# IK2277/ultimate-tictactoe-alphazero

Hardware: AMD Instinct MI355X
Metric: MCTS simulations/sec (whole node), 4096 games × 50 sims/move; 1/2/4/8 GPU (higher is better)
Workload: dtype f32 activations and accumulation; tower point GEMMs as 3-term split-f16 products on the f16 MFMA (f32-level accuracy: within 1e-5 of the reference's fp32 network); 1 GPU; 4096 concurrent self-play games per GPU x 50 sims/move, MCTS_BATCH_SIZE 8, tau 1.0, continuous self-play (finished games refilled; population aged 300 moves before warmup); one step = one move of every game; games_per_gpu=4096, sims_per_move=50, mcts_batch_size=8, aged_moves=300, eval_cache_log2=23, eval_cache_clear_every=0, lanes_per_gpu=2

## Files before the change

include/uttt_nn.h:

```cpp
#ifndef UTTT_NN_H
#define UTTT_NN_H

#include <stdint.h>

#include "uttt_engine.h"

#ifdef __cplusplus
extern "C" {
#endif

#define UTTT_HEAD_PCONV_W 0
#define UTTT_HEAD_PCONV_B (UTTT_HEAD_PCONV_W + 2 * 128)
#define UTTT_HEAD_VCONV_W (UTTT_HEAD_PCONV_B + 2)
#define UTTT_HEAD_VCONV_B (UTTT_HEAD_VCONV_W + 128)
#define UTTT_HEAD_PFC_W (UTTT_HEAD_VCONV_B + 1)
#define UTTT_HEAD_PFC_B (UTTT_HEAD_PFC_W + 81 * 162)
#define UTTT_HEAD_VFC1_W (UTTT_HEAD_PFC_B + 81)
#define UTTT_HEAD_VFC1_B (UTTT_HEAD_VFC1_W + 256 * 81)
#define UTTT_HEAD_VFC2_W (UTTT_HEAD_VFC1_B + 256)
#define UTTT_HEAD_VFC2_B (UTTT_HEAD_VFC2_W + 256)
#define UTTT_HEAD_SIZE (UTTT_HEAD_VFC2_B + 1)

int uttt_nn_stem(uttt_engine_t *eng, const float *w, const float *b, float *out);
int uttt_nn_stem_states(const uttt_state_t *states, int32_t n, const float *w, const float *b, float *out,
                        void *stream);
int uttt_nn_heads(const float *act, const float *head_weights, int32_t n, float *policy, float *value,
                  int32_t softmax, void *stream);
int uttt_nn_heads_dev(const float *act, const float *head_weights, const int32_t *n_dev, int32_t max_n,
                      float *policy, float *value, int32_t softmax, void *stream);

int uttt_nn_wino3h_weights(const float *w, uint16_t *u, float *u_scale);
int uttt_nn_conv3x3_wino3h(const float *x, const uint16_t *u, float u_scale, const float *bias,
                           const float *residual, float *y, const uint32_t *x_amax, int32_t x_amax_per_board,
                           uint32_t *y_amax, uint32_t *amax_clear, int32_t clear_count, int32_t n_boards,
                           void *stream);
int uttt_nn_conv3x3_wino3h_dev(const float *x, const uint16_t *u, float u_scale, const float *bias,
                               const float *residual, float *y, const uint32_t *x_amax, int32_t x_amax_per_board,
                               uint32_t *y_amax, uint32_t *amax_clear, int32_t clear_count, const int32_t *n_dev,
                               int32_t max_boards, void *stream);
int uttt_nn_conv3x3_wino3h_f16(const float *x, const uint16_t *u, float u_scale, const float *bias,
                               const float *residual, float *y, const uint32_t *x_amax, int32_t x_amax_per_board,
                               uint32_t *y_amax, uint32_t *amax_clear, int32_t clear_count, int32_t n_boards,
                               void *stream);
int uttt_nn_conv3x3_wino3h_f16_dev(const float *x, const uint16_t *u, float u_scale, const float *bias,
                                   const float *residual, float *y, const uint32_t *x_amax, int32_t x_amax_per_board,
                                   uint32_t *y_amax, uint32_t *amax_clear, int32_t clear_count, const int32_t *n_dev,
                                   int32_t max_boards, void *stream);
int uttt_nn_tower_wino3h_dev(float *act, int64_t act_stride, const uint16_t *u_all, const float *u_scale_all,
                             const float *bias_all, int32_t n_layers, const uint32_t *stem_amax, uint32_t *rows,
                             int32_t row_stride, uint32_t *ctl, int32_t parity, const int32_t *n_dev,
                             int32_t max_boards, void *stream);
int32_t uttt_nn_tower_ctl_words(int32_t max_boards);
int uttt_nn_wino3h_set_split(int32_t split);
int uttt_nn_amax(const float *x, int64_t count, uint32_t *amax, void *stream);

#ifdef __cplusplus
}
#endif

#endif
```

ultimate-tictactoe-alphazero_amd/csrc/wino3h_conv.hip:

```cpp
#include <hip/hip_runtime.h>

#include <cmath>
#include <cstdint>

#include "uttt_nn.h"
#include "wino3h_impl.h"

namespace uttt {
void set_error(const char *fmt, ...);
}

namespace uttt {
namespace wino3h {
__global__ __launch_bounds__(256) void k_amax(const float *__restrict__ x, int64_t count, uint32_t *__restrict__ amax) {
    float m = 0.0f;
    for (int64_t i = (int64_t)blockIdx.x * 256 + threadIdx.x; i < count; i += (int64_t)gridDim.x * 256)
        m = fmaxf(m, fabsf(x[i]));
#pragma unroll
    for (int off = 32; off > 0; off >>= 1) m = fmaxf(m, __shfl_xor(m, off));
    if ((threadIdx.x & 63) == 0) atomicMax(amax, __builtin_bit_cast(uint32_t, m));
}

}
}
// ... 5 lines not shown
int uttt_nn_wino3h_weights(const float *w, uint16_t *u, float *u_scale) {
    if (!w || !u || !u_scale) {
        set_error("uttt_nn_wino3h_weights: null pointer");
        return UTTT_ERR_ARG;
    }
    static const double G[5][3] = {{0.5, 0, 0},
                                   {-0.5, -0.5, -0.5},
                                   {-1.0 / 6, 1.0 / 6, -1.0 / 6},
                                   {1.0 / 6, 1.0 / 3, 2.0 / 3},
                                   {0, 0, 1}};
    using namespace wino3h;
    double *U = new double[(size_t)NP * C * C];
    double umax = 0.0;
    for (int co = 0; co < C; ++co)
        for (int ci = 0; ci < C; ++ci) {
            const float *g = w + ((size_t)co * C + ci) * 9;
            double tg[5][3];
            for (int p = 0; p < 5; ++p)
                for (int k = 0; k < 3; ++k)
                    tg[p][k] = G[p][0] * g[0 * 3 + k] + G[p][1] * g[1 * 3 + k] + G[p][2] * g[2 * 3 + k];
            for (int p = 0; p < 5; ++p)
                for (int q = 0; q < 5; ++q) {
                    const double v = tg[p][0] * G[q][0] + tg[p][1] * G[q][1] + tg[p][2] * G[q][2];
                    U[((size_t)(p * 5 + q) * C + ci) * C + co] = v;
                    umax = fabs(v) > umax ? fabs(v) : umax;
                }
        }
    if (!std::isfinite(umax)) {
        delete[] U;
        set_error("uttt_nn_wino3h_weights: non-finite weights");
        return UTTT_ERR_ARG;
    }
    int e = 0;
    if (umax > 0.0) {
        frexp(umax, &e);
        e = 15 - e;
    }
    const double su = ldexp(1.0, e);
    for (int xi = 0; xi < NP; ++xi)
        for (int ci = 0; ci < C; ++ci)
            for (int co = 0; co < C; ++co) {
                const double v = U[((size_t)xi * C + ci) * C + co] * su;
                const _Float16 hi = (_Float16)v;
                const _Float16 lo = (_Float16)(v - (double)hi);
                const size_t o = ((size_t)xi * NCH + ci / KC) * 2 * C * 32 +
                                 ((((co / 16) * 4 + (ci % KC) / 8) * 16 + co % 16) * 8 + ci % 8);
                u[o] = __builtin_bit_cast(uint16_t, hi);
                u[o + C * 4 * 8] = __builtin_bit_cast(uint16_t, lo);
            }
    delete[] U;
    *u_scale = (float)su;
    return UTTT_OK;
}

static int conv3x3_wino3h(const float *x, const uint16_t *u, float u_scale, const float *bias, const float *residual,
                          float *y, const uint32_t *x_amax, int32_t x_amax_per_board, uint32_t *y_amax,
                          uint32_t *amax_clear, int32_t clear_count, int32_t n_boards, const int32_t *n_dev,
                          void *stream, bool f16 = false) {
    if (!x || !u || !bias || !y || !x_amax || n_boards < 0 || x == y || (residual && residual == y) ||
        !(u_scale > 0.0f) || clear_count < 0 || (clear_count > 0 && !amax_clear) ||
        (amax_clear && (amax_clear == y_amax || amax_clear == x_amax))) {
        set_error("uttt_nn_conv3x3_wino3h: bad arguments (x_amax required; output must not alias input or residual; "
                  "the cleared max row must differ from x_amax and y_amax)");
        return UTTT_ERR_ARG;
    }
    if (n_boards == 0 && clear_count == 0) return UTTT_OK;
    const int pb = x_amax_per_board ? 1 : 0;
    const int split = wino3h::split_for(n_boards > 0 ? n_boards : 1);
    if (split > 1) {
        const dim3 sgrid((unsigned)(wino3h::n_sets(n_boards > 0 ? n_boards : 1) * split));
        const hipStream_t s = (hipStream_t)stream;
#define UTTT_WINO3S(RES, SP, R, M)                                                                                 \
    hipLaunchKernelGGL((wino3h::k_wino3s_conv<RES, SP, 3, M>), sgrid, dim3(64 * (8 / SP)), 0, s, x, u, u_scale, bias, R, \
                       y, x_amax, pb, y_amax, amax_clear, clear_count, n_boards, n_dev)
        if (f16) {
            if (residual) UTTT_WINO3S(true, 2, residual, wino3h::kF16);
            else UTTT_WINO3S(false, 2, nullptr, wino3h::kF16);
        } else {
            if (residual) UTTT_WINO3S(true, 2, residual, 0);
            else UTTT_WINO3S(false, 2, nullptr, 0);
        }
#undef UTTT_WINO3S
        hipError_t r = hipGetLastError();
        if (r != hipSuccess) {
            set_error("k_wino3s_conv launch: %s", hipGetErrorString(r));
            return UTTT_ERR_HIP;
        }
        return UTTT_OK;
    }
    const dim3 grid(wino3h::grid_size(n_boards > 0 ? n_boards : 1));
    const hipStream_t st = (hipStream_t)stream;
    using wino3h::k_wino3h_conv;
    if (f16) {
        if (residual)
            hipLaunchKernelGGL((k_wino3h_conv<true, wino3h::kF16>), grid, dim3(wino3h::NT), 0, st, x, u, u_scale, bias,
                               residual, y, x_amax, pb, y_amax, amax_clear, clear_count, n_boards, n_dev);
        else
            hipLaunchKernelGGL((k_wino3h_conv<false, wino3h::kF16>), grid, dim3(wino3h::NT), 0, st, x, u, u_scale, bias,
                               nullptr, y, x_amax, pb, y_amax, amax_clear, clear_count, n_boards, n_dev);
    } else if (residual) {
        hipLaunchKernelGGL(k_wino3h_conv<true>, grid, dim3(wino3h::NT), 0, st, x, u, u_scale, bias, residual, y, x_amax,
                           pb, y_amax, amax_clear, clear_count, n_boards, n_dev);
    } else {
        hipLaunchKernelGGL(k_wino3h_conv<false>, grid, dim3(wino3h::NT), 0, st, x, u, u_scale, bias, nullptr, y, x_amax,
                           pb, y_amax, amax_clear, clear_count, n_boards, n_dev);
    }
    hipError_t r = hipGetLastError();
    if (r != hipSuccess) {
        set_error("k_wino3h_conv launch: %s", hipGetErrorString(r));
        return UTTT_ERR_HIP;
    }
    return UTTT_OK;
}

int uttt_nn_conv3x3_wino3h(const float *x, const uint16_t *u, float u_scale, const float *bias, const float *residual,
                           float *y, const uint32_t *x_amax, int32_t x_amax_per_board, uint32_t *y_amax,
                           uint32_t *amax_clear, int32_t clear_count, int32_t n_boards, void *stream) {
    return conv3x3_wino3h(x, u, u_scale, bias, residual, y, x_amax, x_amax_per_board, y_amax, amax_clear, clear_count,
                          n_boards, nullptr, stream);
}

int uttt_nn_conv3x3_wino3h_dev(const float *x, const uint16_t *u, float u_scale, const float *bias,
                               const float *residual, float *y, const uint32_t *x_amax, int32_t x_amax_per_board,
                               uint32_t *y_amax, uint32_t *amax_clear, int32_t clear_count, const int32_t *n_dev,
                               int32_t max_boards, void *stream) {
    if (!n_dev) {
        set_error("uttt_nn_conv3x3_wino3h_dev: n_dev required");
        return UTTT_ERR_ARG;
    }
    return conv3x3_wino3h(x, u, u_scale, bias, residual, y, x_amax, x_amax_per_board, y_amax, amax_clear, clear_count,
                          max_boards, n_dev, stream);
}

int uttt_nn_conv3x3_wino3h_f16(const float *x, const uint16_t *u, float u_scale, const float *bias,
                               const float *residual, float *y, const uint32_t *x_amax, int32_t x_amax_per_board,
                               uint32_t *y_amax, uint32_t *amax_clear, int32_t clear_count, int32_t n_boards,
                               void *stream) {
    return conv3x3_wino3h(x, u, u_scale, bias, residual, y, x_amax, x_amax_per_board, y_amax, amax_clear, clear_count,
                          n_boards, nullptr, stream, true);
}

int uttt_nn_conv3x3_wino3h_f16_dev(const float *x, const uint16_t *u, float u_scale, const float *bias,
                                   const float *residual, float *y, const uint32_t *x_amax, int32_t x_amax_per_board,
                                   uint32_t *y_amax, uint32_t *amax_clear, int32_t clear_count, const int32_t *n_dev,
                                   int32_t max_boards, void *stream) {
    if (!n_dev) {
        set_error("uttt_nn_conv3x3_wino3h_f16_dev: n_dev required");
        return UTTT_ERR_ARG;
    }
    return conv3x3_wino3h(x, u, u_scale, bias, residual, y, x_amax, x_amax_per_board, y_amax, amax_clear, clear_count,
                          max_boards, n_dev, stream, true);
}

int uttt_nn_tower_wino3h_dev(float *act, int64_t act_stride, const uint16_t *u_all, const float *u_scale_all,
                             const float *bias_all, int32_t n_layers, const uint32_t *stem_amax, uint32_t *rows,
                             int32_t row_stride, uint32_t *ctl, int32_t parity, const int32_t *n_dev,
                             int32_t max_boards, void *stream) {
    if (!act || act_stride < (int64_t)max_boards * 81 * 128 || !u_all || !u_scale_all || !bias_all || !stem_amax ||
        !rows || !ctl || n_layers <= 0 || n_layers % 4 != 0 || max_boards < 0 || row_stride < max_boards ||
        (parity != 0 && parity != 1)) {
        set_error("uttt_nn_tower_wino3h_dev: bad arguments (three activation buffers of max_boards boards act_stride "
                  "floats apart, n_layers a positive multiple of 4, row_stride >= max_boards, parity 0 or 1)");
        return UTTT_ERR_ARG;
    }
    if (max_boards == 0) return UTTT_OK;
    static int items = -1, cus = 0;
    if (items < 0) {
        const char *e = getenv("UTTT_TOWER_ITEMS");
        items = (e && *e) ? atoi(e) : 0;
        if (items < 0) items = 0;
        int dev = 0;
        if (hipGetDevice(&dev) != hipSuccess ||
            hipDeviceGetAttribute(&cus, hipDeviceAttributeMultiprocessorCount, dev) != hipSuccess || cus <= 0)
            cus = 256;
        const char *g = getenv("UTTT_TOWER_CUS");
        if (g && *g && atoi(g) > 0 && atoi(g) < cus) cus = atoi(g);
    }
    const int max_items = n_layers * wino3h::n_sets(max_boards);
    int per = items, wgs;
    if (per == 0) {
        wgs = max_items < cus ? max_items : cus;
        per = 1 << 30;
    } else {
        wgs = (max_items + per - 1) / per;
    }
    hipLaunchKernelGGL((wino3h::k_wino3t_tower<wino3h::kHandoff>), dim3((unsigned)wgs), dim3(wino3h::NT), 0,
                       (hipStream_t)stream, act, (int64_t)act_stride, u_all, u_scale_all, bias_all, (int)n_layers,
                       stem_amax, rows, (int)row_stride, ctl, (int)uttt_nn_tower_ctl_words(row_stride), (int)parity, per,
                       (int)max_boards, n_dev);
    hipError_t r = hipGetLastError();
    if (r != hipSuccess) {
        set_error("k_wino3t_tower launch: %s", hipGetErrorString(r));
        return UTTT_ERR_HIP;
    }
    return UTTT_OK;
}

int32_t uttt_nn_tower_ctl_words(int32_t max_boards) {
    const int32_t w = wino3h::kTowerCtlDone + (max_boards + wino3h::GB - 1) / wino3h::GB;
    return (w + 31) / 32 * 32;
}

int uttt_nn_wino3h_set_split(int32_t split) {
    if (split < -1 || split > 2) {
        set_error("uttt_nn_wino3h_set_split: split must be -1 (automatic), 0/1 (the persistent kernel) or 2");
        return UTTT_ERR_ARG;
    }
    wino3h::g_split = split;
    return UTTT_OK;
}

int uttt_nn_amax(const float *x, int64_t count, uint32_t *amax, void *stream) {
    if (!x || !amax || count < 0) {
        set_error("uttt_nn_amax: bad arguments");
        return UTTT_ERR_ARG;
    }
    if (count == 0) return UTTT_OK;
    int64_t blocks = (count + 255) / 256;
    if (blocks > 1024) blocks = 1024;
    hipLaunchKernelGGL(wino3h::k_amax, dim3((unsigned)blocks), dim3(256), 0, (hipStream_t)stream, x, count, amax);
    hipError_t r = hipGetLastError();
    if (r != hipSuccess) {
        set_error("k_amax launch: %s", hipGetErrorString(r));
        return UTTT_ERR_HIP;
    }
    return UTTT_OK;
}

}
```

ultimate-tictactoe-alphazero_amd/uttt_amd/_lib.py:

```python
import ctypes
import os

import numpy as np

PKG_ROOT = os.path.dirname(os.path.dirname(os.path.abspath(__file__)))
LIB_PATH = os.environ.get("UTTT_ENGINE_LIB") or os.path.join(PKG_ROOT, "libuttt_engine.so")

UTTT_OK = 0
ERRORS = {-1: "UTTT_ERR_ARG", -2: "UTTT_ERR_HIP", -3: "UTTT_ERR_CAPACITY", -4: "UTTT_ERR_ORDER",
          -5: "UTTT_ERR_NODEVICE", -6: "UTTT_ERR_NONFINITE"}

KERNELS = {"select": 0, "apply": 1, "encode": 2, "scan": 3, "move_end": 4, "hash_eval": 5, "playout": 15, "solve": 16,
           "solve_leaves": 17,
           "select_levels": 6, "select_trees": 7, "select_max_levels_sum": 9,
           "select_trips": 10, "select_max_trips_sum": 12}


class UtttState(ctypes.Structure):

    _fields_ = [("own", ctypes.c_uint32 * 3), ("opp", ctypes.c_uint32 * 3), ("mains", ctypes.c_uint32),
                ("active", ctypes.c_int32)]


STATE_DTYPE = np.dtype([("own", "<u4", (3,)), ("opp", "<u4", (3,)), ("mains", "<u4"), ("active", "<i4")])
assert STATE_DTYPE.itemsize == ctypes.sizeof(UtttState) == 32

_P = ctypes.c_void_p
_I32 = ctypes.c_int32
_I64 = ctypes.c_int64
_F32 = ctypes.c_float
_I32P = ctypes.POINTER(ctypes.c_int32)
_I64P = ctypes.POINTER(ctypes.c_int64)
_F32P = ctypes.POINTER(ctypes.c_float)
_F64P = ctypes.POINTER(ctypes.c_double)
_U32P = ctypes.POINTER(ctypes.c_uint32)
_U64 = ctypes.c_uint64
_I8P = ctypes.POINTER(ctypes.c_int8)
_SP = ctypes.POINTER(UtttState)

SIGNATURES = {
    "uttt_last_error": (ctypes.c_char_p, []),
    "uttt_version": (ctypes.c_char_p, []),
    "uttt_state_initial": (None, [_SP]),
    "uttt_state_from_arrays": (ctypes.c_int, [_I32P, _I32P, _I32P, _I32P, _I32, _SP]),
    "uttt_state_to_arrays": (None, [_SP, _I32P, _I32P, _I32P, _I32P, _I32P]),
    "uttt_state_next": (ctypes.c_int, [_SP, _I32, _SP]),
    "uttt_state_legal_actions": (ctypes.c_int, [_SP, _I32P]),
    "uttt_state_is_lose": (ctypes.c_int, [_SP]),
    "uttt_state_is_draw": (ctypes.c_int, [_SP]),
    "uttt_state_is_done": (ctypes.c_int, [_SP]),
    "uttt_state_is_first_player": (ctypes.c_int, [_SP]),
    "uttt_state_input_hwc": (None, [_SP, _F32P]),
    "uttt_states_input_hwc": (ctypes.c_int, [_SP, _I64, _F32P]),
    "uttt_state_to_string": (ctypes.c_int, [_SP, ctypes.c_char_p, _I32]),
    "uttt_boltzman": (ctypes.c_int, [_F32P, _I32, _F32, _F32P]),
    "uttt_playout_host": (ctypes.c_int, [_SP, _I64, _I32, _U64, _I32P, _I32P]),
    "uttt_solve_host": (ctypes.c_int, [_SP, _I64, _I32, _I8P, _I8P, _I8P, _I64P, _I8P]),
    "uttt_solve_overlay_host": (ctypes.c_int, [_SP, _I64, _I32, _I32, _I32, _F32P, _I64, _F32P, _I64, _I8P]),
    "uttt_engine_create": (ctypes.c_int, [_I32, _I32, _I32, ctypes.POINTER(_P)]),
    "uttt_engine_destroy": (ctypes.c_int, [_P]),
    "uttt_engine_share_cache": (ctypes.c_int, [_P, _P]),
    "uttt_engine_own_stream": (ctypes.c_int, [_P, ctypes.POINTER(ctypes.c_void_p)]),
    "uttt_engine_set_stream": (ctypes.c_int, [_P, _P]),
    "uttt_engine_device_bytes": (ctypes.c_int64, [_P]),
    "uttt_search_begin": (ctypes.c_int, [_P, _SP, _I32, _I32, _I32]),
    "uttt_search_begin_mode": (ctypes.c_int, [_P, _SP, _I32, _I32, _I32, _I32]),
    "uttt_search_select": (ctypes.c_int, [_P, _P, _I32P]),
    "uttt_search_select_async": (ctypes.c_int, [_P]),
    "uttt_selfplay_move_begin_async": (ctypes.c_int, [_P]),
    "uttt_selfplay_move_end_async": (ctypes.c_int, [_P]),
    "uttt_selfplay_move_result": (ctypes.c_int, [_P, _I64P, _I32P]),
    "uttt_search_count_copy": (ctypes.c_int, [_P, _P]),
    "uttt_search_select_async_tag": (ctypes.c_int, [_P, ctypes.c_int32, ctypes.c_int32]),
    "uttt_search_count_ring": (ctypes.c_int, [_P, _P, _P]),
    "uttt_search_count_ptr": (ctypes.c_int, [_P, ctypes.POINTER(ctypes.c_void_p)]),
    "uttt_search_pending": (ctypes.c_int, [_P, _SP, _I32P]),
    "uttt_search_apply": (ctypes.c_int, [_P, _P, _I64, _P, _I64, _I32, _I32]),
    "uttt_eval_hash": (ctypes.c_int, [_P, _P, _I32, _P, _P]),
    "uttt_eval_hash_dev": (ctypes.c_int, [_P, _P, _P]),
    "uttt_eval_playout_dev": (ctypes.c_int, [_P, _I32, _U64, _P, _P]),
    "uttt_playouts": (ctypes.c_int, [_P, _SP, _I32, _I32, _U64, _I32P, _I32P]),
    "uttt_solve": (ctypes.c_int, [_P, _SP, _I64, _I32, _I8P, _I8P, _I8P, _I64P, _I8P]),
    "uttt_eval_solve_dev": (ctypes.c_int, [_P, _I32, _I32, _I32, _P, _I64, _P, _I64, _P]),
    "uttt_round_hash_async": (ctypes.c_int, [_P, ctypes.c_int32, ctypes.c_int32, _P, _P]),
    "uttt_rounds_hash_async": (ctypes.c_int, [_P, ctypes.c_int32, ctypes.c_int32, _P, _P, ctypes.c_int32]),
    "uttt_rounds_hash_move": (ctypes.c_int, [_P, ctypes.c_int32, ctypes.c_int32, _P, _P, ctypes.c_int32, _P, _P, _P]),
    "uttt_search_select_host": (ctypes.c_int, [_P, _P, _P, _P]),
    "uttt_search_apply_host": (ctypes.c_int, [_P, _P, ctypes.c_int64, _P, ctypes.c_int32]),
    "uttt_search_root_visits": (ctypes.c_int, [_P, _I32P, _I32P]),
    "uttt_search_scores": (ctypes.c_int, [_P, _F32, _F32P, _I32P]),
    "uttt_selfplay_begin": (ctypes.c_int, [_P, _I64, _I64, ctypes.c_uint32, _F32, _I32, _I32, _I64]),
    "uttt_selfplay_move_begin": (ctypes.c_int, [_P, _I32P]),
    "uttt_selfplay_move_end": (ctypes.c_int, [_P, _I64P]),
    "uttt_selfplay_get_rng": (ctypes.c_int, [_P, _I32, _U32P, _I32P]),
    "uttt_selfplay_set_rng": (ctypes.c_int, [_P, _I32, _U32P, _I32]),
    "uttt_selfplay_games": (ctypes.c_int, [_P, _I64P, _I64P, _I32P, _I64, _I64P]),
    "uttt_selfplay_plies": (ctypes.c_int, [_P, _SP, _F64P, ctypes.POINTER(ctypes.c_int8),
                                           ctypes.POINTER(ctypes.c_int8), _F32P, _I64, _I64P]),
    "uttt_engine_set_timing": (ctypes.c_int, [_P, _I32]),
    "uttt_engine_kernel_stats": (ctypes.c_int, [_P, _I32, ctypes.POINTER(ctypes.c_double), _I64P, _I64P]),
    "uttt_engine_reset_stats": (ctypes.c_int, [_P]),
    "uttt_engine_set_cache": (ctypes.c_int, [_P, _I32, _I32]),
    "uttt_engine_cache_clear": (ctypes.c_int, [_P]),
    "uttt_engine_cache_stats": (ctypes.c_int, [_P, _I64P, _I64P, _I64P]),
    "uttt_engine_cache_stats2": (ctypes.c_int, [_P, _I64P, _I64P, _I64P, _I64P]),
    "uttt_nn_stem": (ctypes.c_int, [_P, _P, _P, _P]),
    "uttt_nn_stem_states": (ctypes.c_int, [_P, _I32, _P, _P, _P, _P]),
    "uttt_nn_heads": (ctypes.c_int, [_P, _P, _I32, _P, _P, _I32, _P]),
    "uttt_nn_heads_dev": (ctypes.c_int, [_P, _P, _P, _I32, _P, _P, _I32, _P]),
    "uttt_nn_wino3h_weights": (ctypes.c_int, [_F32P, _P, ctypes.POINTER(ctypes.c_float)]),
    "uttt_nn_conv3x3_wino3h": (ctypes.c_int, [_P, _P, ctypes.c_float, _P, _P, _P, _P, _I32, _P, _P, _I32, _I32, _P]),
    "uttt_nn_conv3x3_wino3h_dev": (ctypes.c_int, [_P, _P, ctypes.c_float, _P, _P, _P, _P, _I32, _P, _P, _I32, _P, _I32,
                                                  _P]),
    "uttt_nn_conv3x3_wino3h_f16": (ctypes.c_int, [_P, _P, ctypes.c_float, _P, _P, _P, _P, _I32, _P, _P, _I32, _I32,
                                                  _P]),
    "uttt_nn_conv3x3_wino3h_f16_dev": (ctypes.c_int, [_P, _P, ctypes.c_float, _P, _P, _P, _P, _I32, _P, _P, _I32, _P,
                                                      _I32, _P]),
    "uttt_nn_tower_wino3h_dev": (ctypes.c_int, [_P, _I64, _P, _P, _P, _I32, _P, _P, _I32, _P, _I32, _P, _I32, _P]),
    "uttt_nn_tower_ctl_words": (ctypes.c_int32, [_I32]),
    "uttt_nn_amax": (ctypes.c_int, [_P, _I64, _P, _P]),
    "uttt_nn_wino3h_set_split": (ctypes.c_int, [_I32]),
}

_lib = None


class EngineError(RuntimeError):
    pass


def load():
    global _lib
    if _lib is None:
        import torch
        if not os.path.exists(LIB_PATH):
            raise ImportError(f"{LIB_PATH} not built: run `make -C {PKG_ROOT}` (or __graft_entry__.build())")
        lib = ctypes.CDLL(LIB_PATH)
        for name, (res, args) in SIGNATURES.items():
            fn = getattr(lib, name)
            fn.restype = res
            fn.argtypes = args
        _lib = lib
    return _lib


_diag = None


def load_diag():
    global _diag
    if _diag is None:
        load()
        path = os.path.join(os.path.dirname(LIB_PATH), "libuttt_diag.so")
        if not os.path.exists(path):
            raise ImportError(f"{path} not built: run `make -C {PKG_ROOT} diag`")
        _diag = ctypes.CDLL(path)
    return _diag


def check(rc):
    if rc != UTTT_OK:
        msg = load().uttt_last_error().decode(errors="replace")
        if rc == -1:
            raise ValueError(msg)
        raise EngineError(f"{ERRORS.get(rc, rc)}: {msg}")
    return rc


def ptr(a, ctype):
    return a.ctypes.data_as(ctypes.POINTER(ctype))
```

ultimate-tictactoe-alphazero_amd/uttt_amd/nnfast.py:

```python
import ctypes
import weakref

import torch

from . import _lib
from ._lib import check
from .engine import RoundCount
from .model import fold_bn

HEAD = {}


def _head_layout():
    if not HEAD:
        o = 0
        for name, size in (("pconv_w", 2 * 128), ("pconv_b", 2), ("vconv_w", 128), ("vconv_b", 1),
                           ("pfc_w", 81 * 162), ("pfc_b", 81), ("vfc1_w", 256 * 81), ("vfc1_b", 256),
                           ("vfc2_w", 256), ("vfc2_b", 1)):
            HEAD[name] = (o, size)
            o += size
        HEAD["size"] = o
    return HEAD


def pack_heads(net, device):
    lay = _head_layout()
    buf = torch.zeros(lay["size"], dtype=torch.float32)
    pw, pb = fold_bn(net.policy_conv, net.policy_bn)
    vw, vb = fold_bn(net.value_conv, net.value_bn)
    parts = {"pconv_w": pw.reshape(-1), "pconv_b": pb, "vconv_w": vw.reshape(-1), "vconv_b": vb,
             "pfc_w": net.policy_fc.weight.t().reshape(-1), "pfc_b": net.policy_fc.bias,
             "vfc1_w": net.value_fc1.weight.t().reshape(-1), "vfc1_b": net.value_fc1.bias,
             "vfc2_w": net.value_fc2.weight.reshape(-1), "vfc2_b": net.value_fc2.bias}
    for k, v in parts.items():
        o, n = lay[k]
        assert v.numel() == n, (k, v.numel(), n)
        buf[o:o + n] = v.detach().float().cpu()
    return buf.to(device)


def _p(t):
    return ctypes.c_void_p(t.data_ptr())


_WEIGHTS = weakref.WeakKeyDictionary()


def _fingerprint(net):
    return tuple((t.data_ptr(), t._version) for t in net.state_dict().values())


@torch.no_grad()
def _prepared_weights(net, dev, conv):
    fp = _fingerprint(net)
    per = _WEIGHTS.setdefault(net, {})
    key = (str(dev), conv)
    hit = per.get(key)
    if hit is not None and hit[0] == fp:
        return hit[1]
    sw, sb = fold_bn(net.conv_input, net.bn_input)
    out = {"stem_w": sw.permute(1, 2, 3, 0).reshape(27, 128).contiguous().to(dev),
           "stem_b": sb.contiguous().to(dev), "heads": pack_heads(net, dev), "wino": []}
    us, sus, bs = [], [], []
    for b in net.residual_blocks:
        for cv, bn in ((b.conv1, b.bn1), (b.conv2, b.bn2)):
            w, bb = fold_bn(cv, bn)
            u, su = wino3h_weights(w)
            us.append(u)
            sus.append(su)
            bs.append(bb.float())
    out["u_all"] = torch.stack(us).to(dev)
    out["bias_all"] = torch.stack(bs).contiguous().to(dev)
    out["scale_all"] = torch.tensor(sus, dtype=torch.float32, device=dev)
    for i in range(0, len(us), 2):
        out["wino"].append(((out["u_all"][i], sus[i], out["bias_all"][i]),
                            (out["u_all"][i + 1], sus[i + 1], out["bias_all"][i + 1])))
    out["stem_bound"] = float(torch.relu(out["stem_b"].double().cpu() +
                                         out["stem_w"].double().cpu().clamp_min(0).sum(0)).max())
    per[key] = (fp, out)
    return out


class FusedNetworkEvaluator:
    needs_input = False
    device_count = True
    NROW = 4

    def __init__(self, net, engine=None, max_batch=None, conv="wino3h", device=None, precision=None, tower=None):
        import os
        net = net.eval()
        if conv != "wino3h":
            raise ValueError("conv must be 'wino3h' (the split-f16 Winograd tower; the f32-MFMA kernel was retired)")
        self.conv = conv
        self.precision = precision or os.environ.get("UTTT_NN_PRECISION", "f32")
        if self.precision not in ("f32", "f16"):
            raise ValueError("precision must be 'f32' (split-f16, f32-level) or 'f16' (one f16 product)")
        self.engine = engine
        self.lib = _lib.load()
        if engine is not None:
            dev = torch.device("cuda", engine.device)
            self.max_batch = max_batch or engine.max_trees
            if self.max_batch < engine.max_trees:
                raise ValueError(f"max_batch {self.max_batch} < the engine's {engine.max_trees} trees")
        else:
            dev = torch.device(device) if device is not None else torch.device("cuda", torch.cuda.current_device())
            if max_batch is None:
                raise ValueError("max_batch is required without an engine")
            self.max_batch = max_batch
        self.device = dev
        self.nconv = 2 * len(net.residual_blocks)
        if self.nconv % self.NROW:
            raise ValueError("the max-row rotation needs a multiple of 4 convolutions")
        w = _prepared_weights(net, dev, conv)
        self.stem_w, self.stem_b, self.heads, self.wino = w["stem_w"], w["stem_b"], w["heads"], w["wino"]
        self.u_all, self.bias_all, self.scale_all = w["u_all"], w["bias_all"], w["scale_all"]
        self.tower = tower or os.environ.get("UTTT_NN_TOWER", "layers")
        if self.tower not in ("dataflow", "layers"):
            raise ValueError("tower must be 'dataflow' (one persistent launch) or 'layers' (a launch per conv)")
        if self.precision == "f16":
            self.tower = "layers"
        self.act = torch.zeros((3, self.max_batch, 81, 128), dtype=torch.float32, device=dev)
        self.buf = [self.act[0], self.act[1], self.act[2]]
        self.ctl = torch.zeros(2 * self.lib.uttt_nn_tower_ctl_words(self.max_batch), dtype=torch.int32, device=dev)
        self.ctl_parity = 0
        self.stem_bound = w["stem_bound"]
        self.stem_amax = torch.tensor([self.stem_bound], dtype=torch.float32, device=dev).view(torch.int32)
        self.bamax = torch.zeros((self.NROW, self.max_batch), dtype=torch.int32, device=dev)
        self.policy = torch.zeros((self.max_batch, 81), dtype=torch.float32, device=dev)
        self.value = torch.zeros((self.max_batch,), dtype=torch.float32, device=dev)
        self.states = None
        self.tower_events = None

    def _stream(self):
        return ctypes.c_void_p(torch.cuda.current_stream(self.device).cuda_stream)

    @torch.no_grad()
    def forward(self, n, softmax=True):
        check(self.lib.uttt_nn_stem(self.engine.h, _p(self.stem_w), _p(self.stem_b), _p(self.buf[0])))
        if isinstance(n, RoundCount):
            return self._tower_heads(n, softmax, n_dev=self.engine.count_ptr())
        return self._tower_heads(n, softmax)

    @torch.no_grad()
    def forward_states(self, states, softmax=True):
        import numpy as np
        n = len(states)
        if n > self.max_batch:
            raise ValueError(f"{n} states > max_batch {self.max_batch}")
        if self.states is None:
            self.states = torch.zeros((self.max_batch, 8), dtype=torch.int32, device=self.device)
        if n == 0:
            return self.policy[:0], self.value[:0]
        st = np.ascontiguousarray(states).view(np.int32).reshape(n, 8)
        self.states[:n].copy_(torch.from_numpy(st))
        check(self.lib.uttt_nn_stem_states(_p(self.states), n, _p(self.stem_w), _p(self.stem_b), _p(self.buf[0]),
                                           self._stream()))
        return self._tower_heads(n, softmax)

    def _dev_plan(self, stream, n_dev):
        key = (stream.value, n_dev.value)
        if getattr(self, "_plan", None) is None or self._plan[0] != key:
            rows = [ctypes.c_void_p(self.bamax[r].data_ptr()) for r in range(self.NROW)]
            cap = self.max_batch
            x, t, y = (ctypes.c_void_p(b.data_ptr()) for b in self.buf)
            calls, i = [], 0
            for (u1, s1, b1), (u2, s2, b2) in self.wino:
                src = (_p(self.stem_amax), 0) if i == 0 else (rows[(i - 1) % 4], 1)
                calls.append((x, _p(u1), ctypes.c_float(s1), _p(b1), None, t, src[0], src[1], rows[i % 4],
                              rows[(i + 1) % 4], cap, n_dev, cap, stream))
                i += 1
                calls.append((t, _p(u2), ctypes.c_float(s2), _p(b2), x, y, rows[(i - 1) % 4], 1, rows[i % 4],
                              rows[(i + 1) % 4], cap, n_dev, cap, stream))
                i += 1
                x, y = y, x
            heads = (x, _p(self.heads), n_dev, cap, _p(self.policy), _p(self.value))
            self._plan = (key, calls, heads)
        return self._plan

    def _tower_dataflow(self, stream, n_dev, max_boards):
        check(self.lib.uttt_nn_tower_wino3h_dev(_p(self.act), ctypes.c_int64(self.act[0].numel()), _p(self.u_all),
                                                _p(self.scale_all), _p(self.bias_all), self.nconv, _p(self.stem_amax),
                                                _p(self.bamax), self.max_batch, _p(self.ctl), self.ctl_parity, n_dev,
                                                int(max_boards), stream))
        self.ctl_parity ^= 1

    def _tower_heads(self, n, softmax, n_dev=None):
        stream = self._stream()
        if self.tower == "dataflow" and (n_dev is not None or n > 28):
            if self.tower_events is not None:
                ev0, ev1 = torch.cuda.Event(enable_timing=True), torch.cuda.Event(enable_timing=True)
                ev0.record()
            self._tower_dataflow(stream, n_dev, self.max_batch if n_dev is not None else n)
            if self.tower_events is not None:
                ev1.record()
                self.tower_events.append((n, ev0, ev1))
            if n_dev is not None:
                check(self.lib.uttt_nn_heads_dev(_p(self.buf[0]), _p(self.heads), n_dev, self.max_batch,
                                                 _p(self.policy), _p(self.value), 1 if softmax else 0, stream))
                return self.policy, self.value
            check(self.lib.uttt_nn_heads(_p(self.buf[0]), _p(self.heads), n, _p(self.policy), _p(self.value),
                                         1 if softmax else 0, stream))
            return self.policy[:n], self.value[:n]
        if n_dev is not None:
            _, calls, heads = self._dev_plan(stream, n_dev)
            if self.tower_events is not None:
                ev0, ev1 = torch.cuda.Event(enable_timing=True), torch.cuda.Event(enable_timing=True)
                ev0.record()
            fn = self.lib.uttt_nn_conv3x3_wino3h_f16_dev if self.precision == "f16" else \
                self.lib.uttt_nn_conv3x3_wino3h_dev
            for a in calls:
                check(fn(*a))
            if self.tower_events is not None:
                ev1.record()
                self.tower_events.append((n, ev0, ev1))
            check(self.lib.uttt_nn_heads_dev(*heads, 1 if softmax else 0, stream))
            return self.policy, self.value
        x, t, y = self.buf
        if self.tower_events is not None:
            ev0, ev1 = torch.cuda.Event(enable_timing=True), torch.cuda.Event(enable_timing=True)
            ev0.record()
        rows = [ctypes.c_void_p(self.bamax[r].data_ptr()) for r in range(self.NROW)]
        cap = self.max_batch
        fn = self.lib.uttt_nn_conv3x3_wino3h_f16 if self.precision == "f16" else self.lib.uttt_nn_conv3x3_wino3h
        i = 0
        for (u1, s1, b1), (u2, s2, b2) in self.wino:
            src = (_p(self.stem_amax), 0) if i == 0 else (rows[(i - 1) % 4], 1)
            check(fn(_p(x), _p(u1), ctypes.c_float(s1), _p(b1), None, _p(t), src[0], src[1], rows[i % 4],
                     rows[(i + 1) % 4], cap, n, stream))
            i += 1
            check(fn(_p(t), _p(u2), ctypes.c_float(s2), _p(b2), _p(x), _p(y), rows[(i - 1) % 4], 1, rows[i % 4],
                     rows[(i + 1) % 4], cap, n, stream))
            i += 1
            x, y = y, x
        if self.tower_events is not None:
            ev1.record()
            self.tower_events.append((n, ev0, ev1))
        check(self.lib.uttt_nn_heads(_p(x), _p(self.heads), n, _p(self.policy), _p(self.value),
                                     1 if softmax else 0, stream))
        return self.policy[:n], self.value[:n]

    def __call__(self, x, n):
        return self.forward(n, True)


def wino3h_weights(w):
    import numpy as np
    wc = np.ascontiguousarray(w.detach().float().cpu().numpy())
    u = np.zeros((25 * 128 * 128 * 2,), np.uint16)
    su = ctypes.c_float(0.0)
    lib = _lib.load()
    check(lib.uttt_nn_wino3h_weights(wc.ctypes.data_as(ctypes.POINTER(ctypes.c_float)),
                                     ctypes.c_void_p(u.ctypes.data), ctypes.byref(su)))
    return torch.from_numpy(u.view(np.int16)), su.value


def set_conv_split(split):
    check(_lib.load().uttt_nn_wino3h_set_split(int(split)))


def amax(x, out=None):
    if out is None:
        out = torch.zeros(1, dtype=torch.int32, device=x.device)
    check(_lib.load().uttt_nn_amax(_p(x), x.numel(), _p(out), ctypes.c_void_p(torch.cuda.current_stream().cuda_stream)))
    return out


def board_amax(x):
    return x.abs().reshape(x.shape[0], -1).amax(dim=1).contiguous().view(torch.int32)


def conv3x3_wino3h(x, u, su, bias, residual=None, y_amax=None, x_amax=None, precision="f32"):
    y = torch.empty_like(x)
    xa = board_amax(x) if x_amax is None else x_amax
    lib = _lib.load()
    fn = lib.uttt_nn_conv3x3_wino3h_f16 if precision == "f16" else lib.uttt_nn_conv3x3_wino3h
    check(fn(_p(x), _p(u), ctypes.c_float(su), _p(bias), _p(residual) if residual is not None else None, _p(y), _p(xa),
             1, _p(y_amax) if y_amax is not None else None, None, 0, x.shape[0],
             ctypes.c_void_p(torch.cuda.current_stream().cuda_stream)))
    return y


_DUAL_ATTRS = ("conv_input", "bn_input", "residual_blocks", "policy_conv", "policy_bn", "policy_fc", "value_conv",
               "value_bn", "value_fc1", "value_fc2")


def is_dual_network(model):
    try:
        if not all(hasattr(model, a) for a in _DUAL_ATTRS) or getattr(model, "training", False):
            return False
        if tuple(model.conv_input.weight.shape) != (128, 3, 3, 3):
            return False
        blocks = list(model.residual_blocks)
        if not blocks or (2 * len(blocks)) % FusedNetworkEvaluator.NROW:
            return False
        for b in blocks:
            if tuple(b.conv1.weight.shape) != (128, 128, 3, 3) or tuple(b.conv2.weight.shape) != (128, 128, 3, 3):
                return False
        return (tuple(model.policy_fc.weight.shape) == (81, 162) and tuple(model.value_fc1.weight.shape) == (256, 81)
                and tuple(model.value_fc2.weight.shape) == (1, 256))
    except (AttributeError, TypeError):
        return False


def evaluator_kind(model, kind=None):
    import os
    kind = kind or os.environ.get("UTTT_EVALUATOR", "auto")
    if kind not in ("auto", "fused", "torch"):
        raise ValueError("evaluator kind must be 'auto', 'fused' or 'torch'")
    if kind == "auto":
        return "fused" if is_dual_network(model) else "torch"
    if kind == "fused" and not is_dual_network(model):
        raise ValueError("the fused evaluator needs a DualNetwork (128 filters, 3x3, eval mode)")
    return kind
```

ultimate-tictactoe-alphazero_amd/uttt_amd/selfplay.py:

```python
import collections
import contextlib
import math
import os
import time

import numpy as np
import torch

from .engine import Engine, RoundCount, initial_states


def _bucket(n, cap, quantum=256):
    if n <= 64:
        b = 1 << max(0, math.ceil(math.log2(max(n, 1))))
    else:
        b = ((n + quantum - 1) // quantum) * quantum
    return min(b, cap)


class HashEvaluator:

    device_count = True
    cheap = True

# ... 65 lines not shown
        self._ring = torch.full((self.kRing, engine.max_trees), -1, dtype=torch.int8, device=dev)
        self._used = 0
        self._totals = torch.zeros(3, dtype=torch.int64, device=dev)
        self.status = self._ring[0]
        torch.cuda.current_stream(dev).synchronize()

    def __call__(self, x, n):
        p, v = self.base(x, n)
        if self._used == self.kRing:
            self._fold()
        self.status = self._ring[self._used]
        self._used += 1
        self.engine.eval_solve_dev(p, v, self.max_empties, self.max_nodes, self.priors, self.status)
        return p, v

    def _fold(self):
        if self._used:
            with torch.cuda.stream(self.engine.stream):
                rows = self._ring[:self._used]
                self._totals += torch.stack([(rows == k).sum() for k in (0, 1, 2)])
                rows.fill_(-1)
            self._used = 0

    def counts(self):
        self._fold()
        with torch.cuda.stream(self.engine.stream):
            k, s, b = self._totals.tolist()
        return {"skipped": k, "solved": s, "budget": b}

    def reset_counts(self):
        self._fold()
        with torch.cuda.stream(self.engine.stream):
            self._totals.zero_()

    @property
    def solved(self):
        return self.counts()["solved"]

    @property
    def budget(self):
        return self.counts()["budget"]

    @property
    def skipped(self):
        return self.counts()["skipped"]


class NetworkEvaluator:

    def __init__(self, model, max_batch):
        self.model = model
        self.max_batch = max_batch

    @torch.no_grad()
    def __call__(self, x, n):
        nb = _bucket(n, self.max_batch)
        p, v = self.model(x[:nb])
        return p[:n].float(), v[:n].float()


def model_evaluator_factory(model, kind=None):
    from .nnfast import FusedNetworkEvaluator, evaluator_kind
    if evaluator_kind(model, kind) == "fused":
        return lambda eng: FusedNetworkEvaluator(model, eng)
    return lambda eng: NetworkEvaluator(model, eng.max_trees)


class BatchedSearch:

    def __init__(self, max_trees, max_sims=50, device=None, cache_log2=0):
        self.engine = Engine(max_trees, max_sims, device)
        if cache_log2:
            self.engine.set_cache(cache_log2, 0)
        dev = torch.device("cuda", self.engine.device)
        self.x = torch.zeros((max_trees, 3, 9, 9), dtype=torch.float32, device=dev)
        self.rounds = 0

    def run(self, roots, evaluator, evaluate_count=50, batch_size=8, semantics="cpp"):
        e = self.engine
        e.use_stream()
        e.search_begin(roots, evaluate_count, batch_size, semantics)
        self.rounds = 0
        x = self.x if getattr(evaluator, "needs_input", True) else None
        while True:
            n = e.select(x)
            if n == 0:
                break
            p, v = evaluator(self.x, n)
            e.apply(p, v)
            self.rounds += 1

    def scores(self, temperature):
        return self.engine.scores(temperature)

    def visits(self):
        return self.engine.root_visits()


class _TagReady:
    __slots__ = ("buf", "tag")

    def __init__(self, buf, tag):
        self.buf, self.tag = buf, tag

    def query(self):
        return int(self.buf[3]) == self.tag


class _Lane:

    def __init__(self, slots, evaluate_count, device, cache_log2, cache_clear_every, own_stream):
        self.engine = Engine(slots, evaluate_count, device)
        if cache_log2:
            self.engine.set_cache(cache_log2, cache_clear_every)
        self.stream = self.engine.own_stream() if own_stream else None
        dev = torch.device("cuda", self.engine.device)
        self.x = torch.zeros((slots, 3, 9, 9), dtype=torch.float32, device=dev)
        self.evaluator = None
        self.rounds = 0
        self.finished = 0
        self.count_ring = None
        self.ring_pos = 0
        self.spec = True
        self._no_rows = None
        self.leaves = 0

    def no_rows(self):
        if self._no_rows is None:
            dev = torch.device("cuda", self.engine.device)
            self._no_rows = (torch.zeros((1, 81), dtype=torch.float32, device=dev),
                             torch.zeros((1,), dtype=torch.float32, device=dev))
        return self._no_rows

    def use_stream(self):
        self.engine.use_stream(self.stream)


class SelfPlay:

    def __init__(self, slots, evaluate_count=50, batch_size=8, temperature=1.0, device=None, evaluator=None,
                 model=None, cache_log2=None, cache_clear_every=0, lanes=1, evaluator_kind=None):
        if lanes < 1 or slots % lanes:
            raise ValueError("slots must be a positive multiple of lanes")
        per = slots // lanes
        if cache_log2 is None:
            cache_log2 = min(23, max(12, int(math.ceil(math.log2(max(per, 1)))) + 11))
        self.lanes = []
        for i in range(lanes):
            self.lanes.append(_Lane(per, evaluate_count, device, cache_log2 if i == 0 else 0, cache_clear_every,
                                    lanes > 1))
            if i and cache_log2:
                self.lanes[i].engine.share_cache(self.lanes[0].engine)
        self.engine = self.lanes[0].engine
        self.x = self.lanes[0].x
        self.slots = slots
        self.evaluate_count = evaluate_count
        self.batch_size = batch_size
        self.temperature = temperature
        if evaluator is None and model is not None:
            self.set_evaluator(model_evaluator_factory(model, evaluator_kind))
        elif evaluator is None:
            self.set_evaluator(HashEvaluator)
        else:
            self.evaluator = evaluator
        self.sims = 0
        self.moves = 0
        self.cache_clear_every = cache_clear_every
        self.async_rounds = os.environ.get("UTTT_ASYNC_ROUNDS", "1") != "0"

    def set_evaluator(self, make):
        for ln in self.lanes:
            ln.evaluator = make(ln.engine)
        self.lanes[0].engine.cache_clear()

    @property
    def evaluator(self):
        return self.lanes[0].evaluator

    @evaluator.setter
    def evaluator(self, ev):
        if len(self.lanes) > 1:
            raise ValueError("with lanes > 1 use set_evaluator(make) (one evaluator per lane)")
        self.lanes[0].evaluator = ev

    @property
    def rounds(self):
        return sum(ln.rounds for ln in self.lanes)

    @property
    def finished(self):
        return sum(ln.finished for ln in self.lanes)

    @property
    def leaves(self):
        return sum(ln.leaves for ln in self.lanes)

    def _ctx(self, ln):
        return torch.cuda.stream(ln.stream) if ln.stream is not None else contextlib.nullcontext()

    def begin(self, game_begin, game_end, seed_base, arena_plies=None):
        n = len(self.lanes)
        span = game_end - game_begin
        for i, ln in enumerate(self.lanes):
            gb = game_begin + span * i // n
            ge = game_begin + span * (i + 1) // n
            if ln.stream is None:
                ln.engine.use_stream()
            else:
                ln.use_stream()
            with self._ctx(ln):
                ln.engine.selfplay_begin(gb, ge, seed_base, self.temperature, self.evaluate_count, self.batch_size,
                                         arena_plies if arena_plies is None else -(-arena_plies // n))
            ln.rounds = ln.finished = 0
        self.sims = self.moves = 0

    def _device_count(self):
        return (self.async_rounds and not self.cache_clear_every and
                all(getattr(ln.evaluator, "device_count", False) for ln in self.lanes))

    def step(self):
        if self._device_count():
            return self.steps(1)
        live = []
        for ln in self.lanes:
            with self._ctx(ln):
                live.append(ln.engine.move_begin())
        active = [ln for ln, n in zip(self.lanes, live) if n > 0]
        if not active:
            return 0
        queue = collections.deque(active)
        while queue:
            ln = queue.popleft()
            e = ln.engine
            with self._ctx(ln):
                x = ln.x if getattr(ln.evaluator, "needs_input", True) else None
                n = e.select(x)
                if n == 0:
                    continue
                p, v = ln.evaluator(ln.x, n)
                e.apply(p, v)
                ln.rounds += 1
            queue.append(ln)
        for ln in active:
            with self._ctx(ln):
                ln.finished = ln.engine.move_end()
        self.moves += 1
        done = sum(live) * self.evaluate_count
        self.sims += done
        return done

    def steps(self, k=None, progress=None):
        if not self._device_count():
            total, i = 0, 0
            while k is None or i < k:
                d = self.step()
                if d == 0:
                    break
                total += d
                i += 1
                if progress:
                    progress(self.finished, None)
            return total
        depth = self._lookahead()
        if (len(self.lanes) == 1 and depth > 1 and os.environ.get("UTTT_MOVE_LOOP", "1") != "0"
                and getattr(self.lanes[0].evaluator, "round_move", None) is not None
                and getattr(self.lanes[0].evaluator, "rounds_per_call", 1) == 1):
            return self._steps_move_loop(self.lanes[0], k, depth, progress)
        spin = depth > 1
        for ln in self.lanes:
            if ln.count_ring is None:
                ln.count_ring = ln.engine.count_ring()
            r = getattr(ln.evaluator, "rounds_per_call", 1)
            if len(ln.count_ring) < (depth + 1) * r and not (r > 1 and len(ln.count_ring) >= depth * r):
                raise ValueError(f"round look-ahead {depth} x {r} rounds per call needs more count slots")

        def fill(ln, q):
            while len(q) < depth:
                q.append(self._enqueue_round(ln, ln.spec if depth == 1 else True))
            return q

        state = {}
        for ln in self.lanes:
            with self._ctx(ln):
                live = ln.engine.move_begin()
            if live > 0:
                ln.cur_live = live
                ln.moves_left = k
                ln.result_pending = False
                state[id(ln)] = (ln, fill(ln, collections.deque()))
        total = moves = 0
        while state:
            ready = [key for key in state if state[key][1][0][1].query()]
            if not ready:
                if not spin:
                    time.sleep(2e-5)
                continue
            for key in ready:
                ln, q = state[key]
                rc, ev, spec, buf = q.popleft()
                if ln.result_pending:
                    ln.finished, ln.cur_live = ln.engine.move_result()
                    ln.result_pending = False
                    if progress:
                        progress(self.finished, None)
                if isinstance(buf, list):
                    n, more = sum(int(b[0]) for b in buf), int(buf[-1][2])
# ... 182 lines not shown
```

Measured before the change: 7.097 million simulations/s.

## Serialize tower launches across lanes with a shared gate and leave CUs free

Adds a shared HIP event gate so that when several self-play lanes run on one GPU, each lane's persistent tower kernel waits for the previous lane's tower to finish. The two persistent dataflow towers therefore no longer contend for CUs or spin against each other. When the gate is active, the tower grid is also capped at the CU count minus a few (default 8) to leave room for MCTS and head kernels to overlap. The cost is that cross-lane overlap of tower work is lost and the tower gets slightly fewer CUs.

```diff
diff --git a/include/uttt_nn.h b/include/uttt_nn.h
--- a/include/uttt_nn.h
+++ b/include/uttt_nn.h
@@ -46,11 +46,17 @@
                                    const float *residual, float *y, const uint32_t *x_amax, int32_t x_amax_per_board,
                                    uint32_t *y_amax, uint32_t *amax_clear, int32_t clear_count, const int32_t *n_dev,
                                    int32_t max_boards, void *stream);
+typedef struct uttt_tower_gate uttt_tower_gate_t;
 int uttt_nn_tower_wino3h_dev(float *act, int64_t act_stride, const uint16_t *u_all, const float *u_scale_all,
                              const float *bias_all, int32_t n_layers, const uint32_t *stem_amax, uint32_t *rows,
                              int32_t row_stride, uint32_t *ctl, int32_t parity, const int32_t *n_dev,
-                             int32_t max_boards, void *stream);
+                             int32_t max_boards, int32_t n_wgs, uttt_tower_gate_t *gate, void *stream);
 int32_t uttt_nn_tower_ctl_words(int32_t max_boards);
+int uttt_nn_tower_gate_create(uttt_tower_gate_t **out);
+int uttt_nn_tower_gate_destroy(uttt_tower_gate_t *gate);
+int uttt_nn_tower_gate_wait(uttt_tower_gate_t *gate, void *stream);
+int uttt_nn_tower_plan(int32_t n_wgs, int32_t cus, int32_t items_cap, int32_t n_layers, int32_t max_boards,
+                       int32_t *wgs, int32_t *max_items);
 int uttt_nn_wino3h_set_split(int32_t split);
 int uttt_nn_amax(const float *x, int64_t count, uint32_t *amax, void *stream);
 
diff --git a/ultimate-tictactoe-alphazero_amd/csrc/wino3h_conv.hip b/ultimate-tictactoe-alphazero_amd/csrc/wino3h_conv.hip
--- a/ultimate-tictactoe-alphazero_amd/csrc/wino3h_conv.hip
+++ b/ultimate-tictactoe-alphazero_amd/csrc/wino3h_conv.hip
@@ -181,10 +181,76 @@
                           max_boards, n_dev, stream, true);
 }
 
+struct uttt_tower_gate {
+    hipEvent_t done = nullptr;
+    bool recorded = false;
+};
+
+int uttt_nn_tower_gate_create(uttt_tower_gate_t **out) {
+    if (!out) {
+        set_error("uttt_nn_tower_gate_create: null pointer");
+        return UTTT_ERR_ARG;
+    }
+    uttt_tower_gate_t *g = new uttt_tower_gate_t;
+    hipError_t r = hipEventCreateWithFlags(&g->done, hipEventDisableTiming);
+    if (r != hipSuccess) {
+        delete g;
+        set_error("uttt_nn_tower_gate_create: %s", hipGetErrorString(r));
+        return UTTT_ERR_HIP;
+    }
+    *out = g;
+    return UTTT_OK;
+}
+
+int uttt_nn_tower_gate_destroy(uttt_tower_gate_t *gate) {
+    if (!gate) return UTTT_OK;
+    (void)hipEventDestroy(gate->done);
+    delete gate;
+    return UTTT_OK;
+}
+
+int uttt_nn_tower_gate_wait(uttt_tower_gate_t *gate, void *stream) {
+    if (!gate || !gate->recorded) return UTTT_OK;
+    hipError_t r = hipStreamWaitEvent((hipStream_t)stream, gate->done, 0);
+    if (r != hipSuccess) {
+        set_error("uttt_nn_tower_gate_wait: %s", hipGetErrorString(r));
+        return UTTT_ERR_HIP;
+    }
+    return UTTT_OK;
+}
+
+static int tower_gate_record(uttt_tower_gate_t *gate, void *stream) {
+    hipError_t r = hipEventRecord(gate->done, (hipStream_t)stream);
+    if (r != hipSuccess) {
+        set_error("uttt_nn_tower_wino3h_dev: recording the gate's event: %s", hipGetErrorString(r));
+        return UTTT_ERR_HIP;
+    }
+    gate->recorded = true;
+    return UTTT_OK;
+}
+
+int uttt_nn_tower_plan(int32_t n_wgs, int32_t cus, int32_t items_cap, int32_t n_layers, int32_t max_boards,
+                       int32_t *wgs, int32_t *max_items) {
+    if (cus <= 0 || items_cap < 0 || n_layers <= 0 || max_boards <= 0 || !wgs || !max_items) {
+        set_error("uttt_nn_tower_plan: bad arguments");
+        return UTTT_ERR_ARG;
+    }
+    const int total = n_layers * wino3h::n_sets(max_boards);
+    if (items_cap == 0) {
+        const int width = n_wgs <= 0 ? cus : (n_wgs < cus ? n_wgs : cus);
+        *wgs = total < width ? total : width;
+        *max_items = 1 << 30;
+    } else {
+        *wgs = (total + items_cap - 1) / items_cap;
+        *max_items = items_cap;
+    }
+    return UTTT_OK;
+}
+
 int uttt_nn_tower_wino3h_dev(float *act, int64_t act_stride, const uint16_t *u_all, const float *u_scale_all,
                              const float *bias_all, int32_t n_layers, const uint32_t *stem_amax, uint32_t *rows,
                              int32_t row_stride, uint32_t *ctl, int32_t parity, const int32_t *n_dev,
-                             int32_t max_boards, void *stream) {
+                             int32_t max_boards, int32_t n_wgs, uttt_tower_gate_t *gate, void *stream) {
     if (!act || act_stride < (int64_t)max_boards * 81 * 128 || !u_all || !u_scale_all || !bias_all || !stem_amax ||
         !rows || !ctl || n_layers <= 0 || n_layers % 4 != 0 || max_boards < 0 || row_stride < max_boards ||
         (parity != 0 && parity != 1)) {
@@ -193,7 +259,7 @@
         return UTTT_ERR_ARG;
     }
     if (max_boards == 0) return UTTT_OK;
-    static int items = -1, cus = 0;
+    static int items = -1, cus = 0, width0 = 0;
     if (items < 0) {
         const char *e = getenv("UTTT_TOWER_ITEMS");
         items = (e && *e) ? atoi(e) : 0;
@@ -203,25 +269,22 @@
             hipDeviceGetAttribute(&cus, hipDeviceAttributeMultiprocessorCount, dev) != hipSuccess || cus <= 0)
             cus = 256;
         const char *g = getenv("UTTT_TOWER_CUS");
-        if (g && *g && atoi(g) > 0 && atoi(g) < cus) cus = atoi(g);
-    }
-    const int max_items = n_layers * wino3h::n_sets(max_boards);
-    int per = items, wgs;
-    if (per == 0) {
-        wgs = max_items < cus ? max_items : cus;
-        per = 1 << 30;
-    } else {
-        wgs = (max_items + per - 1) / per;
-    }
+        width0 = (g && *g && atoi(g) > 0) ? atoi(g) : 0;
+    }
+    int32_t wgs = 0, per = 0;
+    if (uttt_nn_tower_plan(n_wgs > 0 ? n_wgs : width0, cus, items, n_layers, max_boards, &wgs, &per) != UTTT_OK)
+        return UTTT_ERR_ARG;
+    if (gate && uttt_nn_tower_gate_wait(gate, stream) != UTTT_OK) return UTTT_ERR_HIP;
     hipLaunchKernelGGL((wino3h::k_wino3t_tower<wino3h::kHandoff>), dim3((unsigned)wgs), dim3(wino3h::NT), 0,
                        (hipStream_t)stream, act, (int64_t)act_stride, u_all, u_scale_all, bias_all, (int)n_layers,
-                       stem_amax, rows, (int)row_stride, ctl, (int)uttt_nn_tower_ctl_words(row_stride), (int)parity, per,
-                       (int)max_boards, n_dev);
+                       stem_amax, rows, (int)row_stride, ctl, (int)uttt_nn_tower_ctl_words(row_stride), (int)parity,
+                       (int)per, (int)max_boards, n_dev);
     hipError_t r = hipGetLastError();
     if (r != hipSuccess) {
         set_error("k_wino3t_tower launch: %s", hipGetErrorString(r));
         return UTTT_ERR_HIP;
     }
+    if (gate) return tower_gate_record(gate, stream);
     return UTTT_OK;
 }
 
diff --git a/ultimate-tictactoe-alphazero_amd/uttt_amd/_lib.py b/ultimate-tictactoe-alphazero_amd/uttt_amd/_lib.py
--- a/ultimate-tictactoe-alphazero_amd/uttt_amd/_lib.py
+++ b/ultimate-tictactoe-alphazero_amd/uttt_amd/_lib.py
@@ -116,8 +116,13 @@
                                                   _P]),
     "uttt_nn_conv3x3_wino3h_f16_dev": (ctypes.c_int, [_P, _P, ctypes.c_float, _P, _P, _P, _P, _I32, _P, _P, _I32, _P,
                                                       _I32, _P]),
-    "uttt_nn_tower_wino3h_dev": (ctypes.c_int, [_P, _I64, _P, _P, _P, _I32, _P, _P, _I32, _P, _I32, _P, _I32, _P]),
+    "uttt_nn_tower_wino3h_dev": (ctypes.c_int, [_P, _I64, _P, _P, _P, _I32, _P, _P, _I32, _P, _I32, _P, _I32, _I32, _P,
+                                                _P]),
     "uttt_nn_tower_ctl_words": (ctypes.c_int32, [_I32]),
+    "uttt_nn_tower_gate_create": (ctypes.c_int, [ctypes.POINTER(_P)]),
+    "uttt_nn_tower_gate_destroy": (ctypes.c_int, [_P]),
+    "uttt_nn_tower_gate_wait": (ctypes.c_int, [_P, _P]),
+    "uttt_nn_tower_plan": (ctypes.c_int, [_I32, _I32, _I32, _I32, _I32, _I32P, _I32P]),
     "uttt_nn_amax": (ctypes.c_int, [_P, _I64, _P, _P]),
     "uttt_nn_wino3h_set_split": (ctypes.c_int, [_I32]),
 }
diff --git a/ultimate-tictactoe-alphazero_amd/uttt_amd/nnfast.py b/ultimate-tictactoe-alphazero_amd/uttt_amd/nnfast.py
--- a/ultimate-tictactoe-alphazero_amd/uttt_amd/nnfast.py
+++ b/ultimate-tictactoe-alphazero_amd/uttt_amd/nnfast.py
@@ -81,12 +81,34 @@
     return out
 
 
+TOWER_FREE_CUS = 8
+
+
+class TowerGate:
+
+    def __init__(self, device=None):
+        self.lib = _lib.load()
+        h = ctypes.c_void_p()
+        with torch.cuda.device(device if device is not None else torch.cuda.current_device()):
+            check(self.lib.uttt_nn_tower_gate_create(ctypes.byref(h)))
+        self.h = h
+
+    def wait(self, stream):
+        check(self.lib.uttt_nn_tower_gate_wait(self.h, stream))
+
+    def __del__(self):
+        if getattr(self, "h", None):
+            self.lib.uttt_nn_tower_gate_destroy(self.h)
+            self.h = None
+
+
 class FusedNetworkEvaluator:
     needs_input = False
     device_count = True
     NROW = 4
 
-    def __init__(self, net, engine=None, max_batch=None, conv="wino3h", device=None, precision=None, tower=None):
+    def __init__(self, net, engine=None, max_batch=None, conv="wino3h", device=None, precision=None, tower=None,
+                 tower_gate="auto", tower_wgs=None):
         import os
         net = net.eval()
         if conv != "wino3h":
@@ -119,6 +141,17 @@
             raise ValueError("tower must be 'dataflow' (one persistent launch) or 'layers' (a launch per conv)")
         if self.precision == "f16":
             self.tower = "layers"
+        if isinstance(tower_gate, str):
+            if tower_gate != "auto":
+                raise ValueError("tower_gate must be a TowerGate, None or 'auto'")
+            tower_gate = None if os.environ.get("UTTT_TOWER_GATE", "1") == "0" else getattr(engine, "tower_gate", None)
+        self.tower_gate = tower_gate
+        if tower_wgs is None:
+            tower_wgs = 0
+            if tower_gate is not None:
+                free = int(os.environ.get("UTTT_TOWER_FREE_CUS", TOWER_FREE_CUS))
+                tower_wgs = max(1, torch.cuda.get_device_properties(dev).multi_processor_count - free)
+        self.tower_wgs = int(tower_wgs)
         self.act = torch.zeros((3, self.max_batch, 81, 128), dtype=torch.float32, device=dev)
         self.buf = [self.act[0], self.act[1], self.act[2]]
         self.ctl = torch.zeros(2 * self.lib.uttt_nn_tower_ctl_words(self.max_batch), dtype=torch.int32, device=dev)
@@ -181,13 +214,16 @@
         check(self.lib.uttt_nn_tower_wino3h_dev(_p(self.act), ctypes.c_int64(self.act[0].numel()), _p(self.u_all),
                                                 _p(self.scale_all), _p(self.bias_all), self.nconv, _p(self.stem_amax),
                                                 _p(self.bamax), self.max_batch, _p(self.ctl), self.ctl_parity, n_dev,
-                                                int(max_boards), stream))
+                                                int(max_boards), self.tower_wgs,
+                                                self.tower_gate.h if self.tower_gate is not None else None, stream))
         self.ctl_parity ^= 1
 
     def _tower_heads(self, n, softmax, n_dev=None):
         stream = self._stream()
         if self.tower == "dataflow" and (n_dev is not None or n > 28):
             if self.tower_events is not None:
+                if self.tower_gate is not None:
+                    self.tower_gate.wait(stream)
                 ev0, ev1 = torch.cuda.Event(enable_timing=True), torch.cuda.Event(enable_timing=True)
                 ev0.record()
             self._tower_dataflow(stream, n_dev, self.max_batch if n_dev is not None else n)
diff --git a/ultimate-tictactoe-alphazero_amd/uttt_amd/selfplay.py b/ultimate-tictactoe-alphazero_amd/uttt_amd/selfplay.py
--- a/ultimate-tictactoe-alphazero_amd/uttt_amd/selfplay.py
+++ b/ultimate-tictactoe-alphazero_amd/uttt_amd/selfplay.py
@@ -241,6 +241,11 @@
             if i and cache_log2:
                 self.lanes[i].engine.share_cache(self.lanes[0].engine)
         self.engine = self.lanes[0].engine
+        if lanes > 1:
+            from .nnfast import TowerGate
+            gate = TowerGate(self.engine.device)
+            for ln in self.lanes:
+                ln.engine.tower_gate = gate
         self.x = self.lanes[0].x
         self.slots = slots
         self.evaluate_count = evaluate_count
```

Result: no change. 7.089 million simulations/s (-0.1%).
